# Julia-Tempering/Pigeons.jl

Hardware: AMD Instinct MI355X
Metric: replica-steps/sec (explore+swap), toy_mvn d=1024, n_chains=1024; round-trip rate (higher is better)
Workload: dtype f64

## Files before the change

### pigeons.jl_amd/csrc/pte_slice8.hpp

```cpp
#pragma once
#include "pte_slice7.hpp"

namespace pte {

#ifndef PTE_S8_BD
#define PTE_S8_BD 3
#endif
#ifndef PTE_S8_BS
#define PTE_S8_BS 9
#endif
constexpr int S8_BD = PTE_S8_BD;

#ifndef PTE_S8_WAVES
#define PTE_S8_WAVES 4
#endif
template <int NLU, int S8_BS, int WINDOW, int DBL_MODE>
__device__ __forceinline__ void slice8_body(EngineDev e, SliceParams sp, const int64_t cl) {
    using namespace s7;
    constexpr int WIN = WINDOW, REFILL_AT = WINDOW - PTE_S7_MARGIN;
    constexpr bool FAST = (DBL_MODE == 2);
    static_assert(CAP_ITERS >= S8_BS, "lane 0 must be able to run past the speculative budget");
#ifndef PTE_S8_BLK
#define PTE_S8_BLK 256
#endif
    constexpr int BLK = PTE_S8_BLK, CPB = BLK / 64;
    __shared__ struct {
        double u[WIN];
        double e[WIN];
        double x[BLK];
        double we[256];
        unsigned long long ke[256];
    } sm;
    double (&s_u)[WIN] = sm.u; double (&s_e)[WIN] = sm.e; double (&s_x)[BLK] = sm.x; double (&s_we)[256] = sm.we; unsigned long long (&s_ke)[256] = sm.ke;
    const int lane = lane_id();
#ifdef PTE_PROFILE_WAVES
    const uint64_t wave_t0 = __builtin_amdgcn_s_memrealtime();
#endif
    for (int i = lane; i < 256; i += 64) { s_we[i] = ZIG_WE[i]; s_ke[i] = ZIG_KE[i]; }
    __syncthreads();
    if (cl >= e.K) return;
    const int64_t c = e.c0 + cl;
    const int slot = e.slot_of_chain[cl];
    if (is_ref_chain(e, c)) {
        iid_refresh_recorded<NLU>(e, cl, c, slot, e.sd[c], lane);
        return;
    }
    const double lp_before = lp_before_explore(e, c, slot);
    const int64_t d = e.d;
    double *xrow = e.x + (int64_t)slot * e.ld;
    const int B = (int)((d + 63) >> 6);
    const double nhp = e.nhp[c];
    const double inv_nhp = 1.0 / nhp;
    const double inv_abs_nhp = -inv_nhp * (1.0 + 1e-6);
    const double w = sp.w;
    const double w11 = 1.1 * sp.w;
    const int cap_iters = min(sp.max_iter, CAP_ITERS);
    const int kcap = min(sp.p, 20);

    const int hg = s7_level(lane);
    const int hrel = s7_pick(LO, hg, 0) + lane - s7_pick(BASE, hg, 0);

    const int succ_lo = s7_pick(LO, hg + 1, 0), succ_wd = s7_pick(WD, hg + 1, 0), succ_base = s7_pick(BASE, hg + 1, 0);
    const int succ_off = hrel - succ_lo;
    const int word_c = 0x10000 - succ_off;
    const int word_c9 = (1 << 20) - succ_off * 512;
    const uint64_t seed_in = e.rng[2 * slot];

    double BS = 0.0;
    for (int b = 0; b < B; ++b) {
        int64_t i = 64 * (int64_t)b + lane;
        double v = (i < d) ? xrow[i] : 0.0;
        double s = wave_sum_dpp(v * v);
        if (lane == b) BS = s;
    }
    double S = upper_tree_root<NLU>(BS);
    if (nhp * S == -INFINITY) { if (lane == 0) set_error(e, ERR_SLICE_SUPPORT, (int)c, -1); return; }

    uint64_t wseed = e.rng[2 * slot];
    const uint64_t gamma = e.rng[2 * slot + 1];
    int p = 0;
    uint64_t gamma_inv = gamma;
    for (int k = 0; k < 5; ++k) gamma_inv *= 2ull - gamma * gamma_inv;
    double wsum = 0.0;
    auto fill_window = [&]() __attribute__((always_inline)) {
        __syncthreads();
        double acc = 0.0;
#pragma unroll
        for (int k = 0; k < WIN / 64; ++k) {
            const int i = 64 * k + lane;
            const uint64_t r = mix64(wseed + (uint64_t)(i + 1) * gamma);
            const uint64_t ri = r & MASK52;
            const int idx = (int)(ri & 0xFF);
            const bool fast = ri < s_ke[idx];
            const double ev = (double)ri * s_we[idx];
            s_u[i] = u52_to_unit(r);
            s_e[i] = fast ? ev : __longlong_as_double(0x7ff8000000000000LL);
            acc += fast ? ev : 0.0;
        }
        wsum = wave_sum_dpp(acc);
        p = 0;
        __syncthreads();
    };
    fill_window();

    int dbl_z0 = 0, dbl_z1 = 0, dbl_one_hi = 0x3ff00000;
    if constexpr (DBL_MODE == 2) asm volatile("" : "+v"(dbl_z0), "+v"(dbl_z1), "+v"(dbl_one_hi));

    long long steps_sum = 0, fb_draws = 0, ex_total = 0;
    int steps_n = 0, acc_sum = 0, acc_n = 0, n_fb = 0;
    int err = 0, err_coord = -1;
#ifdef PTE_PROFILE_SECTIONS
    long long prof[16] = {0, 0, 0, 0, 0, 0, 0, 0, 0, 0, 0, 0, 0, 0, 0, 0};
#endif

    for (int pass = 0; pass < sp.n_passes && !err; ++pass) {
        for (int b = 0; BLK * (int64_t)b < d && !err; ++b) {
            const int64_t base = BLK * (int64_t)b;
            const int nl = (int)min((int64_t)BLK, d - base);
#pragma unroll
            for (int k = 0; k < CPB; ++k) s_x[64 * k + lane] = (64 * k + lane < nl) ? xrow[base + 64 * k + lane] : 0.0;
            __builtin_amdgcn_wave_barrier();
            double Sest = S * (1.0 + 1e-6) + wsum * inv_abs_nhp;
            int l = 0, l_end = nl;
            do {
                PROF_T(t0);
                if (__builtin_expect(p > REFILL_AT, 0)) { wseed += (uint64_t)p * gamma; fill_window(); Sest = Sest * (1.0 + 1e-6) + wsum * inv_abs_nhp; }
                const bool active = (l + hg) < nl;
                const double xold = s_x[(l + hg) & (BLK - 1)];
                int idx0 = p + hrel;
                double E = s_e[idx0];
                double u0 = s_u[idx0 + 1];
                double Vd[S8_BD];
#pragma unroll
                for (int it = 0; it < S8_BD; ++it) Vd[it] = s_u[idx0 + 2 + it];
                int ex0 = 0;
                int cnt_base = 2;
                if (__builtin_expect((ballot64(E != E) & 1ull) != 0ull, 0)) {
                    SeqRng rs{wseed + (uint64_t)p * gamma, gamma};
                    const double Ex = randexp_seq(rs);
                    const int used = (int)((rs.seed - (wseed + (uint64_t)p * gamma)) * gamma_inv);
                    if (used <= 17) {
                        ex0 = used - 1;
                        if (lane == 0) { E = Ex; idx0 += ex0; cnt_base = 2 + ex0; }
                        Sest += Ex * inv_abs_nhp;
                        ex_total += ex0;
                        u0 = s_u[idx0 + 1];
#pragma unroll
                        for (int it = 0; it < S8_BD; ++it) Vd[it] = s_u[idx0 + 2 + it];
                    }
                }
                const double Enh = E * inv_nhp;
                const double Q = __builtin_fma(xold, xold, -Enh);
                const double Bq = Sest + fabs(Q);
                double dmin = fabs(Enh);
                auto test = [&](double v) __attribute__((always_inline)) -> double {
                    const double d = __builtin_fma(v, v, -Q);
                    dmin = fmin(dmin, fabs(d));
                    return d;
                };
                double LL = xold - w * u0;
                double RR = LL + w;
                double dL = test(LL), dR = test(RR);
                int kd = 0;
                double dmin_lr = 0.0;
#if PTE_S8_BD >= 1 && PTE_S8_BD <= 4 && !defined(PTE_S8_DOUBLING_SELECTS)
                if constexpr (DBL_MODE == 2) {
                    double t_, wd_;
                    int sLh_, sRh_;
                    uint64_t sv_, sx_;
#define PTE_S8_CSTEP(V) \
                    "v_cmp_ge_f64 vcc, 0.5, " V "\n" \
                    "v_min_f64 v[102:103], v[114:115], v[116:117]\n" \
                    "v_cmpx_gt_f64_e64 %[sx], 0, v[102:103]\n" \
                    "v_add_f64 v[112:113], v[98:99], -v[96:97]\n" \
                    "v_add_u32 %[kd], 1, %[kd]\n" \
                    "v_cndmask_b32 v119, 0, %[one], vcc\n" \
                    "v_cndmask_b32 v121, %[one], v118, vcc\n" \
                    "v_fma_f64 v[96:97], -v[118:119], v[112:113], v[96:97]\n" \
                    "v_fma_f64 v[98:99], v[120:121], v[112:113], v[98:99]\n" \
                    "v_fma_f64 v[114:115], v[96:97], v[96:97], -v[110:111]\n" \
                    "v_fma_f64 v[116:117], v[98:99], v[98:99], -v[110:111]\n" \
                    "v_min_f64 v[104:105], v[104:105], |v[114:115]|\n" \
                    "v_min_f64 v[104:105], v[104:105], |v[116:117]|\n"
                    asm volatile("s_mov_b64 %[sv], exec\n"
                                 PTE_S8_CSTEP("%[V0]")
#if PTE_S8_BD >= 2
                                 PTE_S8_CSTEP("%[V1]")
#endif
#if PTE_S8_BD >= 3
                                 PTE_S8_CSTEP("%[V2]")
#endif
#if PTE_S8_BD >= 4
                                 PTE_S8_CSTEP("%[V3]")
#endif
                                 "s_mov_b64 exec, %[sv]\n"
                                 "v_min_f64 v[102:103], v[114:115], v[116:117]\n"
                                 : "+{v[96:97]}"(LL), "+{v[98:99]}"(RR), "+{v[114:115]}"(dL), "+{v[116:117]}"(dR), "+{v[104:105]}"(dmin), [kd] "+v"(kd),
                                   "=&{v[102:103]}"(t_), "=&{v[112:113]}"(wd_), "=&{v119}"(sLh_), "=&{v121}"(sRh_), [sv] "=&s"(sv_), [sx] "=&s"(sx_)
                                 : "{v[110:111]}"(Q), "{v118}"(dbl_z0), "{v120}"(dbl_z1), [one] "v"(dbl_one_hi),
                                   [V0] "v"(Vd[0]), [V1] "v"(Vd[S8_BD > 1 ? 1 : 0]), [V2] "v"(Vd[S8_BD > 2 ? 2 : 0]), [V3] "v"(Vd[S8_BD > 3 ? 3 : 0])
                                 : "vcc", "scc");
#undef PTE_S8_CSTEP
                    dmin_lr = t_;
                } else
                if (DBL_MODE == 1 && sp.p >= S8_BD) {
                    double t_, wd_;
                    uint64_t sv_, sv2_;
#define PTE_S8_DSTEP(V) \
                    "v_min_f64 %[t], %[dL], %[dR]\n" \
                    "v_cmp_gt_f64 vcc, 0, %[t]\n" \
                    "s_and_saveexec_b64 %[sv], vcc\n" \
                    "v_add_u32 %[kd], 1, %[kd]\n" \
                    "v_add_f64 %[wd], %[RR], -%[LL]\n" \
                    "v_cmp_ge_f64 vcc, 0.5, " V "\n" \
                    "s_and_saveexec_b64 %[sv2], vcc\n" \
                    "v_add_f64 %[LL], %[LL], -%[wd]\n" \
                    "v_fma_f64 %[dL], %[LL], %[LL], -%[Q]\n" \
                    "v_min_f64 %[dmin], %[dmin], |%[dL]|\n" \
                    "s_andn2_b64 exec, %[sv2], exec\n" \
                    "v_add_f64 %[RR], %[RR], %[wd]\n" \
                    "v_fma_f64 %[dR], %[RR], %[RR], -%[Q]\n" \
                    "v_min_f64 %[dmin], %[dmin], |%[dR]|\n" \
                    "s_mov_b64 exec, %[sv]\n"
                    asm volatile(PTE_S8_DSTEP("%[V0]")
#if PTE_S8_BD >= 2
                                 PTE_S8_DSTEP("%[V1]")
#endif
#if PTE_S8_BD >= 3
                                 PTE_S8_DSTEP("%[V2]")
#endif
#if PTE_S8_BD >= 4
                                 PTE_S8_DSTEP("%[V3]")
#endif
                                 : [LL] "+v"(LL), [RR] "+v"(RR), [dL] "+v"(dL), [dR] "+v"(dR), [dmin] "+v"(dmin), [kd] "+v"(kd),
                                   [t] "=&v"(t_), [wd] "=&v"(wd_), [sv] "=&s"(sv_), [sv2] "=&s"(sv2_)
                                 : [Q] "v"(Q), [V0] "v"(Vd[0]), [V1] "v"(Vd[S8_BD > 1 ? 1 : 0]), [V2] "v"(Vd[S8_BD > 2 ? 2 : 0]), [V3] "v"(Vd[S8_BD > 3 ? 3 : 0])
                                 : "vcc", "scc");
#undef PTE_S8_DSTEP
                } else
#endif
#pragma unroll
                for (int it = 0; it < S8_BD; ++it) {
                    const bool need = (fmin(dL, dR) < 0.0) && it < sp.p;
                    const double V = Vd[it];
                    kd += need ? 1 : 0;
                    const bool left = V <= 0.5;
                    const double wd = RR - LL;
                    if constexpr (DBL_MODE == 0) {
                        const double sL = (need && left) ? 1.0 : 0.0, sR = (need && !left) ? 1.0 : 0.0;
                        LL = __builtin_fma(-sL, wd, LL);
                        RR = __builtin_fma(sR, wd, RR);
                        dL = __builtin_fma(LL, LL, -Q);
                        dR = __builtin_fma(RR, RR, -Q);
                        dmin = fmin(dmin, fmin(fabs(dL), fabs(dR)));
                    } else {
                        const double cand = left ? (LL - wd) : (RR + wd);
                        const double dc = __builtin_fma(cand, cand, -Q);
                        dmin = need ? fmin(dmin, fabs(dc)) : dmin;
                        const bool nl_ = need && left, nr_ = need && !left;
                        LL = nl_ ? cand : LL;
                        RR = nr_ ? cand : RR;
                        dL = nl_ ? dc : dL;
                        dR = nr_ ? dc : dR;
                    }
                }
#if !(PTE_S8_BD >= 1 && PTE_S8_BD <= 4) || defined(PTE_S8_DOUBLING_SELECTS)
                static_assert(DBL_MODE != 2, "PTE_S8_DBL_MODE == 2 needs the v_cmpx doubling block: 1 <= PTE_S8_BD <= 4 and no PTE_S8_DOUBLING_SELECTS");
#endif
                if constexpr (DBL_MODE != 2) dmin_lr = fmin(dL, dR);
                if (__builtin_expect(ballot64(lane == 0 && (dmin_lr < 0.0) && kd < kcap) != 0ull, 0)) {
                    bool need = (lane == 0);
                    while (need) {
                        const double V = s_u[idx0 + 2 + kd];
                        kd += 1;
                        const bool left = V <= 0.5;
                        const double wd = RR - LL;
                        const double cand = left ? (LL - wd) : (RR + wd);
                        const double dc = test(cand);
                        LL = left ? cand : LL;
                        RR = left ? RR : cand;
                        dL = left ? dc : dL;
                        dR = left ? dR : dc;
                        need = (kd < kcap) && (fmin(dL, dR) < 0.0);
                    }
                    asm volatile("" : "+v"(dL), "+v"(dR), "+v"(kd));
                    dmin_lr = fmin(dL, dR);
                    if constexpr (FAST) dmin_lr = (kd >= sp.p) ? 0.0 : dmin_lr;
                }
                const bool dbl_ok = FAST ? !(dmin_lr < 0.0) : !((kd < sp.p) && (dmin_lr < 0.0));
                double thr2 = 1e-6 * fmax(fabs(LL), fabs(RR));
                if constexpr (DBL_MODE == 2) asm volatile("" : "+v"(thr2));
#ifdef PTE_PROFILE_SECTIONS
                asm volatile("" :: "v"(LL), "v"(RR), "v"(kd), "v"(thr2));
#endif
                PROF_T(t1); PROF_ADD(0, t1 - t0);
                const double *us = &s_u[idx0 + 2 + kd];
                double u[S8_BS];
#pragma unroll
                for (int k = 0; k < S8_BS; ++k) u[k] = us[k];
                double mthr = 2e-12 * Bq;
                int kn0 = cnt_base + kd + succ_off;
                uint64_t pre_ok = ballot64(active && dbl_ok);
                if constexpr (FAST) asm volatile("" : "+v"(mthr), "+v"(kn0), "+s"(pre_ok));
                double Lbar = LL, Rbar = RR, xf = xold, W = 0.0;
                int n = 0;
                bool fin = false;
                uint64_t fin_m = 0ull;
                if constexpr (S8_BS == PTE_S8_BS && S8_BS >= 6 && S8_BS <= 10) {
                    double t_;
                    uint64_t fin_mask, exec_save;
#define PTE_S8_STEP(U) \
                    "v_add_f64 v[112:113], v[98:99], -v[96:97]\n" \
                    "v_mul_f64 v[102:103], " U ", v[112:113]\n" \
                    "v_add_f64 v[100:101], v[96:97], v[102:103]\n" \
                    "v_cmp_lt_f64 vcc, v[100:101], v[108:109]\n" \
                    "v_fma_f64 v[102:103], v[100:101], v[100:101], -v[110:111]\n" \
                    "v_add_u32 v106, 1, v106\n" \
                    "v_cndmask_b32 v96, v96, v100, vcc\n" \
                    "v_cndmask_b32 v97, v97, v101, vcc\n" \
                    "v_cndmask_b32 v98, v100, v98, vcc\n" \
                    "v_cndmask_b32 v99, v101, v99, vcc\n" \
                    "v_min_f64 v[104:105], v[104:105], |v[102:103]|\n" \
                    "v_cmpx_ngt_f64 vcc, 0, v[102:103]\n"
                    asm volatile(".p2align 3\n"
                                 "s_mov_b64 %[sv], exec\n"
                                 PTE_S8_STEP("%[u0]") PTE_S8_STEP("%[u1]") PTE_S8_STEP("%[u2]") PTE_S8_STEP("%[u3]")
                                 PTE_S8_STEP("%[u4]") PTE_S8_STEP("%[u5]")
#if PTE_S8_BS >= 7
                                 PTE_S8_STEP("%[u6]")
#endif
#if PTE_S8_BS >= 8
                                 PTE_S8_STEP("%[u7]")
#endif
#if PTE_S8_BS >= 9
                                 PTE_S8_STEP("%[u8]")
#endif
#if PTE_S8_BS >= 10
                                 PTE_S8_STEP("%[u9]")
#endif
                                 "s_andn2_b64 %[fin], %[sv], exec\n"
                                 "s_mov_b64 exec, %[sv]\n"
                                 "s_nop 3\n"
                                 : "+{v[96:97]}"(Lbar), "+{v[98:99]}"(Rbar), "=&{v[100:101]}"(xf), "=&{v[102:103]}"(t_),
                                   "+{v[104:105]}"(dmin), "+{v106}"(n), "=&{v[112:113]}"(W), [fin] "=&s"(fin_mask), [sv] "=&s"(exec_save)
                                 : "{v[108:109]}"(xold), "{v[110:111]}"(Q), [u0] "v"(u[0]), [u1] "v"(u[1]), [u2] "v"(u[2]), [u3] "v"(u[3]),
                                   [u4] "v"(u[4]), [u5] "v"(u[5]), [u6] "v"(u[S8_BS > 6 ? 6 : 0]), [u7] "v"(u[S8_BS > 7 ? 7 : 0]),
                                   [u8] "v"(u[S8_BS > 8 ? 8 : 0]), [u9] "v"(u[S8_BS > 9 ? 9 : 0])
                                 : "vcc", "scc");
#undef PTE_S8_STEP
                    fin = __builtin_amdgcn_inverse_ballot_w64(fin_mask);
                    fin_m = fin_mask;
                } else {
#pragma unroll
                    for (int k = 0; k < S8_BS; ++k) {
                        W = Rbar - Lbar;
                        const double v = Lbar + u[k] * W;
                        const double dv = __builtin_fma(v, v, -Q);
                        dmin = fmin(dmin, fabs(dv));
                        xf = fin ? xf : v;
                        n += fin ? 0 : 1;
                        const bool below = v < xold;
                        Lbar = below ? v : Lbar;
                        Rbar = below ? Rbar : v;
                        fin = fin || (dv < 0.0);
                    }
                    fin_m = ballot64(fin);
                }
                if (__builtin_expect(ballot64(lane == 0 && !fin && n < cap_iters) != 0ull, 0)) {
                    double dx = 1.0;
                    bool go = (lane == 0);
                    while (go) {
                        W = Rbar - Lbar;
                        xf = Lbar + us[n] * W;
                        n += 1;
                        dx = test(xf);
                        const bool below = xf < xold;
                        Lbar = below ? xf : Lbar;
                        Rbar = below ? Rbar : xf;
                        go = !(dx < 0.0) && n < cap_iters;
                    }
                    asm volatile("" : "+v"(dx), "+v"(n), "+v"(W));
                    fin = fin || (lane == 0 && dx < 0.0);
                    fin_m = ballot64(fin);
                }
                PROF_T(t2); PROF_ADD(1, t2 - t1); PROF_ADD(3, 1);
                int gdone;
#ifdef PTE_PROFILE_SECTIONS
                constexpr bool ASM_TAIL = false;
#else
                constexpr bool ASM_TAIL = FAST && G == 5;
#endif
                if constexpr (ASM_TAIL) {
                    const int kn = kn0 + n;
                    const int wsucc = ((unsigned)kn < (unsigned)succ_wd) ? kn + succ_base : 0;
                    const int word_v = (kn << 9) + word_c9 + wsucc;
                    unsigned acc; uint64_t tmask, sA_, sB_; int w_, pk_, s0_, s1_, s2_, s3_, s4_;
                    asm volatile("v_cmp_gt_f64 vcc, %[W], %[thr]\n"
                                 "v_cndmask_b32_e64 %[w], 0, %[wv], %[pre]\n"
                                 "v_cmp_gt_f64_e64 %[sA], %[dm], %[mthr]\n"
                                 "v_cndmask_b32_e64 %[w], 0, %[w], %[fin]\n"
                                 "v_cndmask_b32_e32 %[w], 0, %[w], vcc\n"
                                 "s_nop 0\n"
                                 "v_cndmask_b32_e64 %[w], 0, %[w], %[sA]\n"
                                 "v_cndmask_b32_e64 %[pk], 0, %[w], %[nz]\n"
                                 : [w] "=&v"(w_), [pk] "=&v"(pk_), [sA] "=&s"(sA_)
                                 : [wv] "v"(word_v), [pre] "s"(pre_ok), [fin] "s"(fin_m), [nz] "s"(0xFFFFFFFFFFFFFFFEull),
                                   [W] "v"(W), [thr] "v"(thr2), [dm] "v"(dmin), [mthr] "v"(mthr)
                                 : "vcc");
                    asm volatile("v_cmp_ne_u32_e64 %[sB], 0, %[w]\n"
                                 "s_mov_b64 %[tm], 1\n"
                                 "v_readlane_b32 %[s0], %[w], 0\n"
                                 "s_nop 3\n"
                                 "v_readlane_b32 %[s1], %[pk], %[s0]\n"
                                 "s_bitset1_b64 %[tm], %[s0]\n"
                                 "s_mov_b32 %[acc], %[s0]\n"
                                 "s_nop 1\n"
                                 "v_readlane_b32 %[s2], %[pk], %[s1]\n"
                                 "s_bitset1_b64 %[tm], %[s1]\n"
                                 "s_add_u32 %[acc], %[acc], %[s1]\n"
                                 "s_nop 1\n"
                                 "v_readlane_b32 %[s3], %[pk], %[s2]\n"
                                 "s_bitset1_b64 %[tm], %[s2]\n"
                                 "s_add_u32 %[acc], %[acc], %[s2]\n"
                                 "s_nop 1\n"
                                 "v_readlane_b32 %[s4], %[pk], %[s3]\n"
                                 "s_bitset1_b64 %[tm], %[s3]\n"
                                 "s_add_u32 %[acc], %[acc], %[s3]\n"
                                 "s_and_b64 %[tm], %[tm], %[sB]\n"
                                 "s_add_u32 %[acc], %[acc], %[s4]\n"
                                 : [sB] "=&s"(sB_), [tm] "=&s"(tmask), [acc] "=&s"(acc),
                                   [s0] "=&s"(s0_), [s1] "=&s"(s1_), [s2] "=&s"(s2_), [s3] "=&s"(s3_), [s4] "=&s"(s4_)
                                 : [w] "v"(w_), [pk] "v"(pk_)
                                 : "scc");
                    if (__builtin_amdgcn_inverse_ballot_w64(tmask)) s_x[(l + hg) & (BLK - 1)] = xf;
                    __builtin_amdgcn_wave_barrier();
                    p += (int)((acc >> 9) & 0x1FFu);
                    gdone = (int)((acc >> 20) & 7u);
                    l += gdone;
                } else {
                bool valid = __builtin_amdgcn_inverse_ballot_w64(pre_ok) && fin && (W > thr2);
                if constexpr (!FAST) valid = valid && !(E != E) && n <= cap_iters;
#ifdef PTE_PROFILE_SECTIONS
                asm volatile("" :: "v"(xf), "v"(n), "v"(dmin));
#endif
#ifdef PTE_PROFILE_SECTIONS
                {
                    const bool mg = dmin > 2e-12 * Bq;
                    const int rc = !active ? 7 : (E != E) ? 1 : !dbl_ok ? 2 : !fin ? 3 : !valid ? 4 : !mg ? 5 : 0;
                    const int cnt_ = cnt_base + kd + n;
                    int o_ = 0, g_ = 0, why = 0;
                    for (g_ = 0; g_ < G; ++g_) {
                        if (l + g_ >= nl) { why = 7; break; }
                        const int k_ = o_ - LO[g_];
                        if ((unsigned)k_ >= (unsigned)WD[g_]) { why = 6; break; }
                        const int ln_ = BASE[g_] + k_;
                        const int r_ = __builtin_amdgcn_readlane(rc, ln_);
                        if (r_) { why = r_; break; }
                        o_ += __builtin_amdgcn_readlane(cnt_, ln_);
                    }
                    PROF_ADD(8 + why, 1);
                }
#endif
                valid = valid && (dmin > mthr);
                const int kn = kn0 + n;
                const bool inw = (unsigned)kn < (unsigned)succ_wd;
                const uint64_t vmask = ballot64(valid);
                int word_v = kn + word_c + (inw ? (int)((unsigned)(kn + succ_base) << 24) : 0);
                asm("" : "+v"(word_v));
                const int word = valid ? word_v : 0;
                const int packed = (lane != 0) ? word : 0;
#ifdef PTE_PROFILE_SECTIONS
                asm volatile("" :: "v"(packed));
#endif
                {
                    int pk = __builtin_amdgcn_readlane(word, 0);
                    unsigned acc = 0u;
                    uint64_t tmask = 1ull;
#pragma unroll
                    for (int g = 1; g < G; ++g) {
                        const int cur = (int)((unsigned)pk >> 24);
                        asm volatile("s_bitset1_b64 %0, %2\n\ts_add_u32 %1, %1, %3" : "+s"(tmask), "+s"(acc) : "s"(cur), "s"(pk) : "scc");
                        pk = __builtin_amdgcn_readlane(packed, cur);
                    }
                    acc += (unsigned)pk;
                    tmask &= vmask;
                    if (__builtin_amdgcn_inverse_ballot_w64(tmask)) s_x[(l + hg) & (BLK - 1)] = xf;
                    __builtin_amdgcn_wave_barrier();
                    p += (int)(acc & 0xFFFFu);
                    gdone = (int)((acc >> 16) & 0xFFu);
                    l += gdone;
                }
                }
#ifdef PTE_PROFILE_SECTIONS
                asm volatile("" :: "s"(p), "s"(l));
#endif
                PROF_T(t4); PROF_ADD(5, t4 - t2); PROF_ADD(4, gdone);
                if (__builtin_expect(gdone == 0, 0)) {
                    ex_total -= ex0;
                    SeqRng rs{wseed + (uint64_t)p * gamma, gamma};
                    const int ck = l >> 6, li = l & 63, bc = CPB * b + ck;
#pragma unroll
                    for (int k = 0; k < CPB; ++k) {
                        const double xk = s_x[64 * k + lane];
                        const double sk = wave_sum_dpp(xk * xk);
                        if (lane == CPB * b + k) BS = sk;
                    }
                    const double X = s_x[64 * ck + lane];
                    const double xo = readlane_f64(X, li);
                    const double E = randexp_seq(rs);
                    const double u0 = rs.rand();
                    const double Q = xo * xo - E * inv_nhp;
                    const double mg = 1e-12 * (Sest + fabs(Q));
                    const double Qlo = Q - mg, Qhi = Q + mg;
                    auto inside_exact = [&](double v) __attribute__((always_inline)) -> bool {
                        const double Xv = (lane == li) ? v : X;
                        const double sv = wave_sum_dpp(Xv * Xv), s0 = wave_sum_dpp(X * X);
                        const double Sv = upper_tree_root<NLU>((lane == bc) ? sv : BS);
                        const double S0 = upper_tree_root<NLU>((lane == bc) ? s0 : BS);
                        const double zz = nhp * S0 - E;
                        return zz < nhp * Sv;
                    };
                    auto inside = [&](double v) __attribute__((always_inline)) -> bool {
                        const double q = v * v;
                        const bool in = q < Qlo;
                        const bool out = q > Qhi;
                        if (__builtin_expect(!(in || out), 0)) return inside_exact(v);
                        return in;
                    };
                    double LL = xo - w * u0;
                    double RR = LL + w;
                    bool in_L = inside(LL), in_R = inside(RR);
                    int K = sp.p;
                    while (K > 0 && (in_L || in_R)) {
                        const double V = rs.rand();
                        if (V <= 0.5) { LL = LL - (RR - LL); in_L = inside(LL); }
                        else { RR = RR + (RR - LL); in_R = inside(RR); }
                        K -= 1;
                    }
                    steps_sum += (sp.p - K); steps_n += 1;
                    const bool doubled = (RR - LL) > w11;
                    double Lbar = LL, Rbar = RR;
                    double xn = xo;
                    bool fin = false;
                    for (int n = 1; n <= sp.max_iter; ++n) {
                        const double newpos = Lbar + rs.rand() * (Rbar - Lbar);
                        if (inside(newpos)) {
                            bool ok = true;
                            if (doubled) {
                                double Lhat = LL, Rhat = RR;
                                bool oL = !in_L, oR = !in_R;
                                bool Rstale = false, Lstale = false, D = false;
                                while (Rhat - Lhat > w11) {
                                    const double Mid = (Lhat + Rhat) / 2.0;
                                    if ((xo < Mid && newpos >= Mid) || (xo >= Mid && newpos < Mid)) D = true;
                                    if (newpos < Mid) { Rhat = Mid; Rstale = true; }
                                    else { Lhat = Mid; Lstale = true; }
                                    if (D) {
                                        if (Lstale) { oL = !inside(Lhat); Lstale = false; }
                                        if (Rstale) { oR = !inside(Rhat); Rstale = false; }
                                        if (oL && oR) { ok = false; break; }
                                    }
                                }
                            }
                            acc_n += 1;
                            if (ok) { acc_sum += 1; xn = newpos; steps_sum += n; steps_n += 1; fin = true; break; }
                        }
                        if (newpos < xo) Lbar = newpos; else Rbar = newpos;
                        if (jl_isapprox(Lbar, Rbar)) { steps_sum += n; steps_n += 1; fin = true; break; }
                    }
                    if (!fin) { err = ERR_SLICE_MAX_ITER; err_coord = (int)(base + l); l_end = 0; continue; }
                    Sest = Sest + fabs(xn * xn - xo * xo);
                    if (lane == li) s_x[l] = xn;
                    __builtin_amdgcn_wave_barrier();
                    l += 1;
                    const int used = (int)((rs.seed - (wseed + (uint64_t)p * gamma)) * gamma_inv);
                    p += used;
                    fb_draws += used; n_fb += 1;
                    PROF_T(t5); PROF_ADD(7, t5 - t4); PROF_ADD(6, 1);
                }
            } while (l < l_end);
            if (err) break;
            {
#pragma unroll
                for (int k = 0; k < CPB; ++k) {
                    const double X = s_x[64 * k + lane];
                    if (64 * k + lane < nl) xrow[base + 64 * k + lane] = X;
                    const double s = wave_sum_dpp(X * X);
                    if (lane == CPB * b + k) BS = s;
                }
                S = upper_tree_root<NLU>(BS);
                if (__builtin_expect(!isfinite(nhp * S), 0)) { err = ERR_SLICE_INVALID_LP; err_coord = (int)base; }
            }
        }
    }
    if (err) { if (lane == 0) set_error(e, err, (int)c, err_coord); return; }
    if (lane == 0) {
        const uint64_t seed_out = wseed + (uint64_t)p * gamma;
        const long long n_spec = (long long)sp.n_passes * d - n_fb;
        const long long spec_draws = (long long)((seed_out - seed_in) * gamma_inv) - fb_draws;
        steps_sum += spec_draws - ex_total - 2 * n_spec; steps_n += (int)(2 * n_spec); acc_sum += (int)n_spec; acc_n += (int)n_spec;
        e.suff[slot] = S;
        e.rng[2 * slot] = seed_out;
        e.expl_steps_sum[cl] += (double)steps_sum; e.expl_steps_n[cl] += steps_n;
        e.expl_acc_sum[cl] += (double)acc_sum;     e.expl_acc_n[cl] += acc_n;
#ifdef PTE_PROFILE_SECTIONS
        for (int i = 0; i < 16; ++i) e.on_m2[16 * cl + i] += (double)prof[i];
#endif
    }
    record_after_explore(e, cl, c, slot, lane, lp_before, S, 0.0);
#ifdef PTE_PROFILE_WAVES
    if (lane == 0) {
        double *o = e.on_m2 + 2 * (e.d + 1) + 4 * cl;
        o[0] = (double)wave_t0; o[1] = (double)__builtin_amdgcn_s_memrealtime();
        o[2] = (double)__builtin_amdgcn_s_getreg((31 << 11) | 4); o[3] = (double)__builtin_amdgcn_s_getreg((31 << 11) | 20);
    }
#endif
}

#ifndef PTE_S8_DBL_MODE
#define PTE_S8_DBL_MODE 2
#endif
template <int NLU, int S8_BS>
__global__ __launch_bounds__(64) __attribute__((amdgpu_waves_per_eu(PTE_S8_WAVES, PTE_S8_WAVES))) void k_explore_slice8(EngineDev e, SliceParams sp) {
    slice8_body<NLU, S8_BS, PTE_S7_WIN, PTE_S8_DBL_MODE>(e, sp, blockIdx.x);
}
template <int NLU, int S8_BS>
__global__ __launch_bounds__(64) __attribute__((amdgpu_waves_per_eu(PTE_S8_WAVES, PTE_S8_WAVES))) void k_explore_slice8_generic(EngineDev e, SliceParams sp) {
    slice8_body<NLU, S8_BS, PTE_S7_WIN, 0>(e, sp, blockIdx.x);
}
#ifndef PTE_S8_TWIN_WAVES
#define PTE_S8_TWIN_WAVES PTE_S8_WAVES
#endif
#ifndef PTE_S8_TWIN_FROM
#define PTE_S8_TWIN_FROM (256 * 8)
#endif
template <int NLU, int S8_BS>
__global__ __launch_bounds__(64) __attribute__((amdgpu_waves_per_eu(PTE_S8_TWIN_WAVES, PTE_S8_TWIN_WAVES))) void k_explore_slice8_lds10k(EngineDev e, SliceParams sp) {
    slice8_body<NLU, S8_BS, 256, 1>(e, sp, blockIdx.x);
}

template <int NLU, int S8_BS, int WINDOW, int DBL_MODE>
__device__ __forceinline__ void slice8_scan_loop(EngineDev e, const SliceParams &sp, const ScanLoop &sl) {
    const int lane = lane_id();
    const int64_t cl = scan_loop_chain(e.K);
    int go = 1;
    if (lane == 0) go = scan_loop_gate(sl) ? 1 : 0;
    if (!__builtin_amdgcn_readfirstlane(go)) return;
    for (int64_t i = 0; i < sl.n_scans; ++i) {
        e.trace_idx = sl.scan_idx0 + i;
        slice8_body<NLU, S8_BS, WINDOW, DBL_MODE>(e, sp, cl);
        __syncthreads();
        int slot = 0;
        if (lane == 0) slot = swap_handshake(e, sl, i, cl, e.slot_of_chain[cl]);
        slot = __builtin_amdgcn_readfirstlane(slot);
        __syncthreads();
        if (slot < 0) return;
    }
}
template <int NLU, int S8_BS>
__global__ __launch_bounds__(64) __attribute__((amdgpu_waves_per_eu(PTE_S8_WAVES, PTE_S8_WAVES))) void k_scans_slice8(EngineDev e, SliceParams sp, ScanLoop sl) {
    slice8_scan_loop<NLU, S8_BS, PTE_S7_WIN, PTE_S8_DBL_MODE>(e, sp, sl);
}
template <int NLU, int S8_BS>
__global__ __launch_bounds__(64) __attribute__((amdgpu_waves_per_eu(PTE_S8_WAVES, PTE_S8_WAVES))) void k_scans_slice8_generic(EngineDev e, SliceParams sp, ScanLoop sl) {
    slice8_scan_loop<NLU, S8_BS, PTE_S7_WIN, 0>(e, sp, sl);
}
}
```

Measured before the change: 1.534 million.

## Keep whole chain row in LDS across passes and defer lane-0 continuation

For small dimensions (NLU<=5), the scan-loop kernel now loads the entire state row into shared memory once per explore. It computes the initial sum of squares from LDS and writes the row back to global memory only at the end, instead of reloading and storing each 256-wide block every pass. The zigguraut tables are loaded into LDS only on the first scan iteration. In the fast ASM-tail mode, the lane-0 continuation loop is deferred to the rare gdone==0 path and retried before falling back. This cuts global traffic and wave-wide ballots, at the cost of more LDS per block (possibly lowering occupancy) and more complex indexing.

```diff
diff --git a/pigeons.jl_amd/csrc/pte_slice8.hpp b/pigeons.jl_amd/csrc/pte_slice8.hpp
--- a/pigeons.jl_amd/csrc/pte_slice8.hpp
+++ b/pigeons.jl_amd/csrc/pte_slice8.hpp
@@ -14,8 +14,8 @@
 #ifndef PTE_S8_WAVES
 #define PTE_S8_WAVES 4
 #endif
-template <int NLU, int S8_BS, int WINDOW, int DBL_MODE>
-__device__ __forceinline__ void slice8_body(EngineDev e, SliceParams sp, const int64_t cl) {
+template <int NLU, int S8_BS, int WINDOW, int DBL_MODE, bool ROW_LDS = false>
+__device__ __forceinline__ void slice8_body(EngineDev e, SliceParams sp, const int64_t cl, const bool tables = true) {
     using namespace s7;
     constexpr int WIN = WINDOW, REFILL_AT = WINDOW - PTE_S7_MARGIN;
     constexpr bool FAST = (DBL_MODE == 2);
@@ -24,19 +24,20 @@
 #define PTE_S8_BLK 256
 #endif
     constexpr int BLK = PTE_S8_BLK, CPB = BLK / 64;
+    constexpr int ROW = ROW_LDS ? ((64 << NLU) > BLK ? (64 << NLU) : BLK) : BLK;
     __shared__ struct {
         double u[WIN];
         double e[WIN];
-        double x[BLK];
+        double x[ROW];
         double we[256];
         unsigned long long ke[256];
     } sm;
-    double (&s_u)[WIN] = sm.u; double (&s_e)[WIN] = sm.e; double (&s_x)[BLK] = sm.x; double (&s_we)[256] = sm.we; unsigned long long (&s_ke)[256] = sm.ke;
+    double (&s_u)[WIN] = sm.u; double (&s_e)[WIN] = sm.e; double (&s_x)[ROW] = sm.x; double (&s_we)[256] = sm.we; unsigned long long (&s_ke)[256] = sm.ke;
     const int lane = lane_id();
 #ifdef PTE_PROFILE_WAVES
     const uint64_t wave_t0 = __builtin_amdgcn_s_memrealtime();
 #endif
-    for (int i = lane; i < 256; i += 64) { s_we[i] = ZIG_WE[i]; s_ke[i] = ZIG_KE[i]; }
+    if (!ROW_LDS || tables) for (int i = lane; i < 256; i += 64) { s_we[i] = ZIG_WE[i]; s_ke[i] = ZIG_KE[i]; }
     __syncthreads();
     if (cl >= e.K) return;
     const int64_t c = e.c0 + cl;
@@ -67,6 +68,23 @@
     const uint64_t seed_in = e.rng[2 * slot];
 
     double BS = 0.0;
+    if constexpr (ROW_LDS) {
+#pragma unroll 1
+        for (int k0 = 0; k0 < ROW / 64; k0 += 4) {
+            double v[4];
+#pragma unroll
+            for (int k = 0; k < 4; ++k) { const int i = 64 * (k0 + k) + lane; v[k] = (i < d) ? xrow[i] : 0.0; }
+#pragma unroll
+            for (int k = 0; k < 4; ++k) s_x[64 * (k0 + k) + lane] = v[k];
+        }
+        __builtin_amdgcn_wave_barrier();
+#pragma unroll 1
+        for (int b = 0; b < B; ++b) {
+            const double v = s_x[64 * b + lane];
+            const double s = wave_sum_dpp(v * v);
+            if (lane == b) BS = s;
+        }
+    } else
     for (int b = 0; b < B; ++b) {
         int64_t i = 64 * (int64_t)b + lane;
         double v = (i < d) ? xrow[i] : 0.0;
@@ -117,16 +135,20 @@
         for (int b = 0; BLK * (int64_t)b < d && !err; ++b) {
             const int64_t base = BLK * (int64_t)b;
             const int nl = (int)min((int64_t)BLK, d - base);
-#pragma unroll
-            for (int k = 0; k < CPB; ++k) s_x[64 * k + lane] = (64 * k + lane < nl) ? xrow[base + 64 * k + lane] : 0.0;
+            const int lb = ROW_LDS ? (int)base : 0;
+            if constexpr (!ROW_LDS) {
+#pragma unroll
+                for (int k = 0; k < CPB; ++k) s_x[64 * k + lane] = (64 * k + lane < nl) ? xrow[base + 64 * k + lane] : 0.0;
+            }
             __builtin_amdgcn_wave_barrier();
             double Sest = S * (1.0 + 1e-6) + wsum * inv_abs_nhp;
-            int l = 0, l_end = nl;
+            int l = lb, l_end = lb + nl;
+            const int l_hi = lb + nl;
             do {
                 PROF_T(t0);
                 if (__builtin_expect(p > REFILL_AT, 0)) { wseed += (uint64_t)p * gamma; fill_window(); Sest = Sest * (1.0 + 1e-6) + wsum * inv_abs_nhp; }
-                const bool active = (l + hg) < nl;
-                const double xold = s_x[(l + hg) & (BLK - 1)];
+                const bool active = (l + hg) < l_hi;
+                const double xold = s_x[(l + hg) & (ROW - 1)];
                 int idx0 = p + hrel;
                 double E = s_e[idx0];
                 double u0 = s_u[idx0 + 1];
@@ -366,7 +388,13 @@
                     }
                     fin_m = ballot64(fin);
                 }
-                if (__builtin_expect(ballot64(lane == 0 && !fin && n < cap_iters) != 0ull, 0)) {
+#ifdef PTE_PROFILE_SECTIONS
+                constexpr bool ASM_TAIL = false;
+#else
+                constexpr bool ASM_TAIL = FAST && G == 5;
+#endif
+                constexpr bool DEFER = ASM_TAIL;
+                auto lane0_continues = [&]() __attribute__((always_inline)) {
                     double dx = 1.0;
                     bool go = (lane == 0);
                     while (go) {
@@ -382,15 +410,13 @@
                     asm volatile("" : "+v"(dx), "+v"(n), "+v"(W));
                     fin = fin || (lane == 0 && dx < 0.0);
                     fin_m = ballot64(fin);
+                };
+                if constexpr (!DEFER) {
+                    if (__builtin_expect(ballot64(lane == 0 && !fin && n < cap_iters) != 0ull, 0)) lane0_continues();
                 }
                 PROF_T(t2); PROF_ADD(1, t2 - t1); PROF_ADD(3, 1);
                 int gdone;
-#ifdef PTE_PROFILE_SECTIONS
-                constexpr bool ASM_TAIL = false;
-#else
-                constexpr bool ASM_TAIL = FAST && G == 5;
-#endif
-                if constexpr (ASM_TAIL) {
+                auto asm_tail = [&]() __attribute__((always_inline)) -> int {
                     const int kn = kn0 + n;
                     const int wsucc = ((unsigned)kn < (unsigned)succ_wd) ? kn + succ_base : 0;
                     const int word_v = (kn << 9) + word_c9 + wsucc;
@@ -432,11 +458,15 @@
                                    [s0] "=&s"(s0_), [s1] "=&s"(s1_), [s2] "=&s"(s2_), [s3] "=&s"(s3_), [s4] "=&s"(s4_)
                                  : [w] "v"(w_), [pk] "v"(pk_)
                                  : "scc");
-                    if (__builtin_amdgcn_inverse_ballot_w64(tmask)) s_x[(l + hg) & (BLK - 1)] = xf;
+                    if (__builtin_amdgcn_inverse_ballot_w64(tmask)) s_x[(l + hg) & (ROW - 1)] = xf;
                     __builtin_amdgcn_wave_barrier();
                     p += (int)((acc >> 9) & 0x1FFu);
-                    gdone = (int)((acc >> 20) & 7u);
-                    l += gdone;
+                    const int g_ = (int)((acc >> 20) & 7u);
+                    l += g_;
+                    return g_;
+                };
+                if constexpr (ASM_TAIL) {
+                    gdone = asm_tail();
                 } else {
                 bool valid = __builtin_amdgcn_inverse_ballot_w64(pre_ok) && fin && (W > thr2);
                 if constexpr (!FAST) valid = valid && !(E != E) && n <= cap_iters;
@@ -484,7 +514,7 @@
                     }
                     acc += (unsigned)pk;
                     tmask &= vmask;
-                    if (__builtin_amdgcn_inverse_ballot_w64(tmask)) s_x[(l + hg) & (BLK - 1)] = xf;
+                    if (__builtin_amdgcn_inverse_ballot_w64(tmask)) s_x[(l + hg) & (ROW - 1)] = xf;
                     __builtin_amdgcn_wave_barrier();
                     p += (int)(acc & 0xFFFFu);
                     gdone = (int)((acc >> 16) & 0xFFu);
@@ -496,16 +526,22 @@
 #endif
                 PROF_T(t4); PROF_ADD(5, t4 - t2); PROF_ADD(4, gdone);
                 if (__builtin_expect(gdone == 0, 0)) {
+                    if constexpr (DEFER) {
+                        if ((pre_ok & 1ull) != 0ull && (fin_m & 1ull) == 0ull && S8_BS < cap_iters) {
+                            lane0_continues();
+                            if (asm_tail() != 0) continue;
+                        }
+                    }
                     ex_total -= ex0;
                     SeqRng rs{wseed + (uint64_t)p * gamma, gamma};
-                    const int ck = l >> 6, li = l & 63, bc = CPB * b + ck;
+                    const int ck = (l - lb) >> 6, li = l & 63, bc = CPB * b + ck;
 #pragma unroll
                     for (int k = 0; k < CPB; ++k) {
-                        const double xk = s_x[64 * k + lane];
+                        const double xk = s_x[lb + 64 * k + lane];
                         const double sk = wave_sum_dpp(xk * xk);
                         if (lane == CPB * b + k) BS = sk;
                     }
-                    const double X = s_x[64 * ck + lane];
+                    const double X = s_x[lb + 64 * ck + lane];
                     const double xo = readlane_f64(X, li);
                     const double E = randexp_seq(rs);
                     const double u0 = rs.rand();
@@ -568,7 +604,7 @@
                         if (newpos < xo) Lbar = newpos; else Rbar = newpos;
                         if (jl_isapprox(Lbar, Rbar)) { steps_sum += n; steps_n += 1; fin = true; break; }
                     }
-                    if (!fin) { err = ERR_SLICE_MAX_ITER; err_coord = (int)(base + l); l_end = 0; continue; }
+                    if (!fin) { err = ERR_SLICE_MAX_ITER; err_coord = (int)(base + (l - lb)); l_end = 0; continue; }
                     Sest = Sest + fabs(xn * xn - xo * xo);
                     if (lane == li) s_x[l] = xn;
                     __builtin_amdgcn_wave_barrier();
@@ -583,8 +619,8 @@
             {
 #pragma unroll
                 for (int k = 0; k < CPB; ++k) {
-                    const double X = s_x[64 * k + lane];
-                    if (64 * k + lane < nl) xrow[base + 64 * k + lane] = X;
+                    const double X = s_x[lb + 64 * k + lane];
+                    if constexpr (!ROW_LDS) if (64 * k + lane < nl) xrow[base + 64 * k + lane] = X;
                     const double s = wave_sum_dpp(X * X);
                     if (lane == CPB * b + k) BS = s;
                 }
@@ -594,6 +630,13 @@
         }
     }
     if (err) { if (lane == 0) set_error(e, err, (int)c, err_coord); return; }
+    if constexpr (ROW_LDS) {
+#pragma unroll 1
+        for (int k0 = 0; k0 < ROW / 64; k0 += 4) {
+#pragma unroll
+            for (int k = 0; k < 4; ++k) { const int i = 64 * (k0 + k) + lane; if (i < d) xrow[i] = s_x[i]; }
+        }
+    }
     if (lane == 0) {
         const uint64_t seed_out = wseed + (uint64_t)p * gamma;
         const long long n_spec = (long long)sp.n_passes * d - n_fb;
@@ -648,7 +691,7 @@
     if (!__builtin_amdgcn_readfirstlane(go)) return;
     for (int64_t i = 0; i < sl.n_scans; ++i) {
         e.trace_idx = sl.scan_idx0 + i;
-        slice8_body<NLU, S8_BS, WINDOW, DBL_MODE>(e, sp, cl);
+        slice8_body<NLU, S8_BS, WINDOW, DBL_MODE, NLU <= 5>(e, sp, cl, i == 0);
         __syncthreads();
         int slot = 0;
         if (lane == 0) slot = swap_handshake(e, sl, i, cl, e.slot_of_chain[cl]);
```

Measured after the change: 1.547 million, median of 6. Within noise of the previous version (+0.9%).
